# minfenli/refnerf-pl

Measured on AMD Instinct MI355X. Metric: ray-samples/s (4096 rays x 128 samples x 2 levels, Ref-NeRF Blender, eval forward), higher is better.
Workload: dtype f16x2; 1 GPU; blender_refnerf.gin, 4096 rays x 128 samples, 2-level, Model.__call__ eval forward with compute_extras + full ray_history; rays_per_gpu=4096, total_rays=4096, samples_per_level=128, parallelism=ray-tile dp1, n_ranks_seen=1, hip_graph_replay=False

## Files before the change

refnerf-pl_amd/csrc/refnerf_device_math.h:

```cpp
#pragma once
#include <hip/hip_runtime.h>

#include "refnerf_detmath.h"
#include "refnerf_layout.h"
#include "refnerf_ide_tables.h"

namespace rn {

constexpr float EPS32 = 1.1920928955078125e-07f;
constexpr float HALF_PI_F = 1.57079637050628662109375f;
constexpr float T100PI = 314.159271240234375f;
constexpr float LOG3_F = 1.09861228466033935546875f;
constexpr float LOG2E_F = 1.44269504088896341f;
constexpr float LN2_F = 0.69314718055994531f;
constexpr float INV_2PI_F = 0.15915494309189535f;


__device__ __forceinline__ float clip01(float x) { return fminf(fmaxf(x, 0.0f), 1.0f); }

__device__ __forceinline__ float s_to_t(float s, float nearv, float farv) {
  float a = s * farv;
  float b = (1.0f - s) * nearv;
  return a + b;
}
// ... 58 lines not shown

__device__ __forceinline__ void cast_sample(const float o[3], const float d[3], float radius, float t0,
                                            float t1, int ray_shape, float lmean[3], float lvar[3]) {
  float t_mean, t_var, r_var;
  frustum_moments(radius, t0, t1, ray_shape, t_mean, t_var, r_var);
  float dms = fmaxf(1e-10f, (d[0] * d[0] + d[1] * d[1]) + d[2] * d[2]);
  float mean[3], cd[3];
#pragma unroll
  for (int i = 0; i < 3; ++i) {
    mean[i] = d[i] * t_mean + o[i];
    float d_outer = d[i] * d[i];
    float null_outer = 1.0f - d[i] * (d[i] / dms);
    cd[i] = t_var * d_outer + r_var * null_outer;
  }
  lmean[0] = -mean[2]; lmean[1] = -mean[1]; lmean[2] = -mean[0];
  lvar[0] = cd[2]; lvar[1] = cd[1]; lvar[2] = cd[0];
}

__device__ __forceinline__ void cast_sample_full(const float o[3], const float d[3], float radius, float t0, float t1, int ray_shape,
                                                 float mean[3], float cov[9]) {
  float t_mean, t_var, r_var;
  frustum_moments(radius, t0, t1, ray_shape, t_mean, t_var, r_var);
  const float dms = fmaxf(1e-10f, (d[0] * d[0] + d[1] * d[1]) + d[2] * d[2]);
#pragma unroll
  for (int i = 0; i < 3; ++i) {
    mean[i] = d[i] * t_mean + o[i];
#pragma unroll
    for (int k = 0; k < 3; ++k) {
      const float d_outer = d[i] * d[k];
      const float null_outer = (i == k ? 1.0f : 0.0f) - d[i] * (d[k] / dms);
      cov[3 * i + k] = t_var * d_outer + r_var * null_outer;
    }
  }
}
__device__ __forceinline__ void lift_onto(const float mean[3], const float cov[9], const float b[3], float &lm, float &lv) {
  lm = fmaf(mean[2], b[2], fmaf(mean[1], b[1], mean[0] * b[0]));
  float acc = 0.0f;
#pragma unroll
  for (int i = 0; i < 3; ++i) {
    const float cb = fmaf(cov[3 * i + 2], b[2], fmaf(cov[3 * i + 1], b[1], cov[3 * i] * b[0]));
    acc = (i == 0) ? b[0] * cb : acc + b[i] * cb;
  }
  lv = acc;
}

__device__ __forceinline__ float safe_arg(float x) {
  if (fabsf(x) < T100PI) return x;
  float m = fmodf(x, T100PI);
  if (m != 0.0f && m < 0.0f) m += T100PI;
  return m;
}

__device__ __forceinline__ void quadrant_reduce(float a, float &r, int &q) {
  const float k = __builtin_rintf(a * 0.636619772367581343f);
  r = fmaf(-k, 7.54978995489188216e-8f, fmaf(-k, 4.837512969970703125e-4f, fmaf(-k, 1.5703125f, a)));
  q = (int)k;
}
__device__ __forceinline__ float sin_reduced(float a) {
  float r; int q;
  quadrant_reduce(a, r, q);
  const float r2 = r * r;
  const float s = fmaf(fmaf(fmaf(-1.9515295891e-4f, r2, 8.3321608736e-3f), r2, -1.6666654611e-1f) * r2, r, r);
  const float c = fmaf(fmaf(fmaf(2.443315711809948e-5f, r2, -1.388731625493765e-3f), r2, 4.166664568298827e-2f) * r2, r2, fmaf(-0.5f, r2, 1.0f));
  const float v = (q & 1) ? c : s;
  return (q & 2) ? -v : v;
}
__device__ __forceinline__ float cos_reduced(float a) {
  float r; int q;
  quadrant_reduce(a, r, q);
  const float r2 = r * r;
  const float s = fmaf(fmaf(fmaf(-1.9515295891e-4f, r2, 8.3321608736e-3f), r2, -1.6666654611e-1f) * r2, r, r);
  const float c = fmaf(fmaf(fmaf(2.443315711809948e-5f, r2, -1.388731625493765e-3f), r2, 4.166664568298827e-2f) * r2, r2, fmaf(-0.5f, r2, 1.0f));
  const float v = (q & 1) ? s : c;
  return ((q + 1) & 2) ? -v : v;
}
__device__ __forceinline__ float safe_arg_exact(float x) {
  const float q = __builtin_floorf(fmaf(x, 1.0f / T100PI, 3e-4f));
  float r = fmaf(-q, T100PI, x);
  r = (r < 0.0f) ? r + T100PI : r;
  return (fabsf(x) < T100PI) ? x : r;
}
__device__ __forceinline__ float ipe_feature_split(float lm, float lv, int j, int cos_block) {
  const float sc = __builtin_ldexpf(1.0f, j), sc2 = __builtin_ldexpf(1.0f, 2 * j);
  float x = lm * sc;
  if (cos_block) x = x + HALF_PI_F;
  const float e = __builtin_amdgcn_exp2f((-0.5f * LOG2E_F) * (lv * sc2));
  return e * sin_reduced(safe_arg_exact(x));
}

template <bool FAST = false>
__device__ __forceinline__ float ipe_feature(float lm, float lv, int j, int cos_block) {
  float sc = __builtin_ldexpf(1.0f, j), sc2 = __builtin_ldexpf(1.0f, 2 * j);
  if (FAST) {
    float r = (lm * sc) * INV_2PI_F;
    if (cos_block) r = r + 0.25f;
    r = __builtin_amdgcn_fractf(r);
    float e = __builtin_amdgcn_exp2f((-0.5f * LOG2E_F) * (lv * sc2));
    return e * __builtin_amdgcn_sinf(r);
  }
  float x = lm * sc;
  if (cos_block) x = x + HALF_PI_F;
  float e = expf(-0.5f * (lv * sc2));
  return e * sinf(safe_arg(x));
}

template <bool FAST> __device__ __forceinline__ float m_exp(float x) {
  if (FAST) return __builtin_amdgcn_exp2f(x * LOG2E_F);
  return expf(x);
}
template <bool FAST> __device__ __forceinline__ float m_log(float x) {
  if (FAST) return __builtin_amdgcn_logf(x) * LN2_F;
  return logf(x);
}
template <bool FAST> __device__ __forceinline__ float m_div(float a, float b) {
  if (FAST) return a * __builtin_amdgcn_rcpf(b);
  return a / b;
}
template <bool FAST> __device__ __forceinline__ float softplus_m(float x) {
  if (FAST) return x > 20.0f ? x : m_log<true>(1.0f + m_exp<true>(x));
  return x > 20.0f ? x : log1pf(expf(x));
}
template <bool FAST> __device__ __forceinline__ float sigmoid_m(float x) { return m_div<FAST>(1.0f, 1.0f + m_exp<FAST>(-x)); }
__device__ __forceinline__ float softplus_t(float x) { return softplus_m<false>(x); }
__device__ __forceinline__ float sigmoid_t(float x) { return sigmoid_m<false>(x); }

template <bool FAST = false>
__device__ __forceinline__ float linear_to_srgb(float x) {
  float srgb0 = (float)(323.0 / 25.0) * x;
  float pw = FAST ? __builtin_amdgcn_exp2f(__builtin_amdgcn_logf(fmaxf(EPS32, x)) * (float)(5.0 / 12.0))
                  : powf(fmaxf(EPS32, x), (float)(5.0 / 12.0));
  float srgb1 = FAST ? (211.0f * pw - 11.0f) * (1.0f / 200.0f) : (211.0f * pw - 11.0f) / 200.0f;
  return (x <= 0.0031308f) ? srgb0 : srgb1;
}

template <bool FAST = false, typename Emit>
__device__ __forceinline__ void ide_eval(float x, float y, float z, float kappa_inv, int part, Emit emit) {
  float att1 = m_exp<FAST>(-1.0f * kappa_inv), att2 = m_exp<FAST>(-3.0f * kappa_inv), att4 = m_exp<FAST>(-10.0f * kappa_inv);
  float att8 = m_exp<FAST>(-36.0f * kappa_inv), att16 = m_exp<FAST>(-136.0f * kappa_inv);
  float pr = 1.0f, pi = 0.0f;
#pragma unroll
  for (int m = 0; m <= 16; ++m) {
    if (m > 0) { float nr = pr * x - pi * y; float ni = pr * y + pi * x; pr = nr; pi = ni; }
    const float pw = part ? pi : pr;
    float tm2 = 0.0f, tm1 = IDE_C[m];
#pragma unroll
    for (int l = m; l <= 16; ++l) {
      float tl;
      if (l == m) tl = IDE_C[m];
      else { tl = IDE_A[m][l] * (z * tm1 - IDE_B[m][l] * tm2); tm2 = tm1; tm1 = tl; }
      if (l == 1) emit(0 + m, pw * (tl * att1));
      if (l == 2) emit(2 + m, pw * (tl * att2));
      if (l == 4) emit(5 + m, pw * (tl * att4));
      if (l == 8) emit(10 + m, pw * (tl * att8));
      if (l == 16) emit(19 + m, pw * (tl * att16));
    }
  }
}

template <bool FAST = false, bool REDUCED = false, typename Emit>
__device__ __forceinline__ void posenc_eval(float x, float y, float z, int part, Emit emit) {
  const float d[3] = {x, y, z};
  const float half_pi = (float)(0.5 * 3.14159265358979323846);
#pragma unroll
  for (int q = 0; q < IDE_TERMS; ++q) {
    float v = 0.0f;
    if (q < 3 && part == 0) v = d[q];
// ... 105 lines not shown
```

refnerf-pl_amd/csrc/refnerf_level_bf16.h:

```cpp
#pragma once
#include <type_traits>

#include "refnerf_level_common.h"

namespace rn {

typedef short v2s __attribute__((ext_vector_type(2)));

struct MmBf16 {
  typedef __bf16 t;
  typedef t v8 __attribute__((ext_vector_type(8)));
  typedef t v2 __attribute__((ext_vector_type(2)));
  static __device__ __forceinline__ v16f mfma(v8 a, v8 b, v16f c) { return __builtin_amdgcn_mfma_f32_32x32x16_bf16(a, b, c, 0, 0, 0); }
};
struct MmF16 {
  typedef _Float16 t;
  typedef t v8 __attribute__((ext_vector_type(8)));
  typedef t v2 __attribute__((ext_vector_type(2)));
  static __device__ __forceinline__ v16f mfma(v8 a, v8 b, v16f c) { return __builtin_amdgcn_mfma_f32_32x32x16_f16(a, b, c, 0, 0, 0); }
};
template <typename MM>
__device__ __forceinline__ unsigned cvt_pk_mm(float lo, float hi) {
  typename MM::v2 r = __builtin_convertvector((v2f){lo, hi}, typename MM::v2);
  return __builtin_bit_cast(unsigned, r);
// ... 338 lines not shown
      RN_STAMPW(A, 3 + phase * 8);

      if (phase == 0) bf_layer<MM, BF_LDS8, BF_IPE_REAL_KS>(p, ar, 0, R0, bn, R0);
      else bf_layer<MM, BF_BNLDS, BF_DIR_REAL_KS>(p, ar, 0, R0, bn, R0);
      RN_STAMPW(A, 4 + phase * 8);
#pragma unroll 1
      for (int it = 0; it < 4; ++it) {
        const int second = (it == 2) ? (phase ? 2 : 1) : 0;
        bf_layer<MM, BF_REG, 0>(p, ar, second, R0, bn, R1);
        if (it < 3) bf_layer<MM, BF_REG, 0>(p, ar, 0, R1, bn, R0);
      }
      RN_STAMPW(A, 5 + phase * 8);
      if (phase == 0) {
#pragma unroll
        for (int ob = 0; ob < 5; ++ob) {
          v16f acc;
          bf_slice<MM, BF_REG, 0>(p, ar, 0, R1, bn, acc);
          if (ob < 4) pack_acc<MM, false>(acc, bn[2 * ob], bn[2 * ob + 1]);
          else {
            int cb = col + 4 * h * BT;
            asm volatile("" : "+v"(cb));
#pragma unroll
            for (int rr = 0; rr < 8; ++rr) {
              int row = (rr & 3) + 8 * (rr >> 2) + 4 * h;
              if (row < HD_ROWS) HD[((rr & 3) + 8 * (rr >> 2)) * BT + cb] = acc[rr];
            }
          }
        }
        wave_sync();
        RN_STAMPW(A, 6);
      } else {
        v16f acc;
        bf_slice<MM, BF_REG, 0>(p, ar, 0, R1, bn, acc);
        float raw_rgb[3];
#pragma unroll
        for (int i = 0; i < 3; ++i) raw_rgb[i] = __shfl(acc[i], n, 64);
        int g_w, rl_w, si_w; bool valid;
        locate(g_w, rl_w, si_w, valid);
        int lane_w = lane, pass_w = pass0;
        asm volatile("" : "+v"(lane_w), "+s"(pass_w));
        if (valid && h == 0) {
          SampleHeads sh;
          load_heads(sh);
          colour_store<ENC_FAST, NPS_EVAL, PSM>(A, sh, raw_rgb, PS, PX, n_tot, g_w, col);
        }
        wave_sync();
        history_flush<NPS_EVAL, PSM>(A, PS, PX, n_tot, pass_w + wave * 32, wave * 32, (size_t)ray0 * N + pass_w + wave * 32, lane_w);
        RN_STAMPW(A, 14);
      }
    }
    __builtin_amdgcn_wave_barrier();
    pass_epilogue();
  }
  asm volatile("s_waitcnt vmcnt(0)" ::: "memory");
  __syncthreads();
  RN_STAMPW(A, 15);
#ifdef REFNERF_PROF_WAITS
  if (A.prof && blockIdx.x == 0 && lane == 0) { A.prof[wave * 32 + 20] = p.t_vm; A.prof[wave * 32 + 21] = p.t_bar; }
#endif

  if constexpr (!RINGPS) composite_phase<BF_NW, true, NPS_EVAL>(A, TD, XP, PS, n_tot, ray0, wave, lane, reinterpret_cast<float *>(WB), NRM);
  RN_STAMPW(A, 16);
}

#ifndef REFNERF_SECONDARY_TU
__global__ __launch_bounds__(BF_NTHREADS) void level_fwd_bf16(const LevelArgs A) { level_fwd_mm<MmBf16>(A); }
__global__ __launch_bounds__(BF_NTHREADS) void level_fwd_f16(const LevelArgs A) { level_fwd_mm<MmF16>(A); }
__global__ __launch_bounds__(BF_NTHREADS) void level_fwd_bf16_ring(const LevelArgs A) { level_fwd_mm<MmBf16, true>(A); }
__global__ __launch_bounds__(BF_NTHREADS) void level_fwd_f16_ring(const LevelArgs A) { level_fwd_mm<MmF16, true>(A); }
#endif

typedef unsigned v2uu __attribute__((ext_vector_type(2)));

__device__ __forceinline__ unsigned pk_f16(float lo, float hi) { return cvt_pk_mm<MmF16>(lo, hi); }
__device__ __forceinline__ void split_pair_f16(float x0, float x1, unsigned &hi, unsigned &lo) {
  hi = pk_f16(x0, x1);
  asm("" : "+v"(hi));
  const MmF16::v2 hv = __builtin_bit_cast(MmF16::v2, hi);
  const _Float16 h0 = hv[0], h1 = hv[1];
  lo = pk_f16(x0 - (float)h0, x1 - (float)h1);
}
typedef _Float16 sq_v8 __attribute__((ext_vector_type(8)));
constexpr int SQ_NF = 4;
struct SqAcc { v4f t0, t1; };
template <int KIND> constexpr int sq_nm() { return KIND == SQ_X ? 18 : (KIND == SQ_BN ? 32 : 24); }
template <int KIND> constexpr int sq_np() { return KIND == SQ_X ? 12 : 16; }
template <int KIND> constexpr int sq_step(int j) { return KIND == SQ_BN ? j / 4 : (KIND == SQ_SC ? j / 3 : j / 6); }
template <int KIND> constexpr int sq_piece(int j) {
  if (KIND == SQ_BN) return 2 * (j / 4) + (j & 1);
  if (KIND == SQ_SC) return 2 * (j / 3) + ((j % 3) == 1 ? 1 : 0);
  return 4 * (j / 6) + ((j % 6) < 4 ? (j % 6) : (j % 6) - 4);
}
template <int KIND> constexpr bool sq_lo(int j) { return KIND == SQ_BN ? (j & 3) >= 2 : (KIND == SQ_SC ? (j % 3) == 2 : (j % 6) >= 4); }
template <int KIND> constexpr int sq_tile(int j) { return KIND == SQ_SC ? 0 : (KIND == SQ_BN ? (j & 1) : ((j % 6) & 1)); }
template <int KIND> constexpr int sq_release(int j) {
  if (KIND == SQ_BN) return (j & 3) >= 2 ? 2 * (j / 4) + ((j & 3) - 2) : -1;
  if (KIND == SQ_SC) return (j % 3) == 1 ? 2 * (j / 3) + 1 : ((j % 3) == 2 ? 2 * (j / 3) : -1);
  const int jj = j % 6, sl = j / 6;
  return jj == 2 ? 4 * sl + 2 : (jj == 3 ? 4 * sl + 3 : (jj == 4 ? 4 * sl : (jj == 5 ? 4 * sl + 1 : -1)));
}
template <int KIND, bool PRE, typename Hook = NoHook>
__device__ __forceinline__ void sq_chunk(Pipe &p, sq_v8 (&fr)[SQ_NF], const v4uu (&in)[16], SqAcc &acc, SqAcc &nacc, Hook &&hook = Hook(), int adv = BF_CHUNK_BYTES) {
  constexpr int NM = sq_nm<KIND>(), NP = sq_np<KIND>();
  constexpr int RDV = NM / 2 - 1;
  const char *w = p.wbuf + p.cur_off;
  const char *cur = w + 1024 + p.lane * 16;
  const char *nxt = p.wbuf + p.nxt_off + 1024 + p.lane * 16;
  sq_v8 xb[2];
  if (KIND == SQ_X) { xb[0] = lds_frag<MmF16>(p.xps); xb[1] = lds_frag<MmF16>(p.xps + (BT / 2) * 16); }
  __builtin_amdgcn_sched_barrier(0);
#pragma unroll
  for (int j = 0; j < NM; ++j) {
    const int sl = sq_step<KIND>(j);
    sq_v8 b;
    if (KIND == SQ_X) b = xb[sq_lo<KIND>(j) ? 1 : 0];
    else b = __builtin_bit_cast(sq_v8, in[2 * ((KIND == SQ_B ? 4 : 0) + sl) + (sq_lo<KIND>(j) ? 1 : 0)]);
    if (sq_tile<KIND>(j)) acc.t1 = __builtin_amdgcn_mfma_f32_16x16x32_f16(fr[sq_piece<KIND>(j) % SQ_NF], b, acc.t1, 0, 0, 0);
    else acc.t0 = __builtin_amdgcn_mfma_f32_16x16x32_f16(fr[sq_piece<KIND>(j) % SQ_NF], b, acc.t0, 0, 0, 0);
    const int rel = sq_release<KIND>(j);
    if (rel >= 0) {
      const int q = rel + SQ_NF;
      fr[rel % SQ_NF] = (q < NP) ? lds_frag<MmF16>(cur + q * 1024) : lds_frag<MmF16>(nxt + (q - NP) * 1024);
    }
    hook(j);
    if (KIND == SQ_X) {
      if ((j % 6) == 3 && sl + 1 < 3) xb[0] = lds_frag<MmF16>(p.xps + (sl + 1) * (4 * BT * 16));
      if ((j % 6) == 5 && sl + 1 < 3) xb[1] = lds_frag<MmF16>(p.xps + (sl + 1) * (4 * BT * 16) + (BT / 2) * 16);
    }
    if (j == RDV) {
      RN_RENDEZVOUS(p);
      issue_chunk<true>(p, p.fil_off, 0);
      if (PRE) {
        const v4f *bp = reinterpret_cast<const v4f *>(p.wbuf + p.nxt_off + (p.lane >> 4) * 16);
        nacc.t0 = bp[0];
        nacc.t1 = bp[4];
      }
    }
    if (j == RDV + 4) issue_chunk<true>(p, p.fil_off, 1);
    if (j == RDV + 8) issue_chunk<true>(p, p.fil_off, 2, adv);
    __builtin_amdgcn_sched_barrier(0);
  }
  ring_rotate(p);
}
__device__ __forceinline__ void sq_epi_piece(const SqAcc &a, int q, v4uu &oh, v4uu &ol) {
  const float y0 = q == 0 ? a.t0[0] : (q == 1 ? a.t0[2] : (q == 2 ? a.t1[0] : a.t1[2]));
  const float y1 = q == 0 ? a.t0[1] : (q == 1 ? a.t0[3] : (q == 2 ? a.t1[1] : a.t1[3]));
  const float x0 = (y0 < 0.0f) ? 0.0f : y0, x1 = (y1 < 0.0f) ? 0.0f : y1;
  unsigned hi, lo;
  split_pair_f16(x0, x1, hi, lo);
  oh[q] = hi;
  ol[q] = lo;
}
template <bool LAYER0>
__device__ __forceinline__ void sq_layer(Pipe &p, sq_v8 (&fr)[SQ_NF], SqAcc (&accs)[2], bool skip, const v4uu (&in)[16], v4uu (&out)[16]) {
#pragma unroll
  for (int ob = 0; ob < 8; ++ob) {
    SqAcc &acc = accs[(ob + 1) & 1];
    SqAcc &prev = accs[ob & 1];
    auto hook = [&](int j) {
      if (ob == 0 || j >= 8 || (j & 1)) return;
      sq_epi_piece(prev, j >> 1, out[2 * ob - 2], out[2 * ob - 1]);
    };
    if constexpr (LAYER0) sq_chunk<SQ_X, true>(p, fr, in, acc, prev, hook);
    else {
      sq_chunk<SQ_A, false>(p, fr, in, acc, prev, hook);
      sq_chunk<SQ_B, true>(p, fr, in, acc, prev);
      if (skip) sq_chunk<SQ_X, true>(p, fr, in, acc, prev);
    }
  }
#pragma unroll
  for (int q = 0; q < 4; ++q) sq_epi_piece(accs[0], q, out[14], out[15]);
  __builtin_amdgcn_sched_barrier(0);
}
__device__ __forceinline__ void sq_bias_now(const Pipe &p, SqAcc &acc) {
  const v4f *bp = reinterpret_cast<const v4f *>(p.wbuf + p.cur_off + (p.lane >> 4) * 16);
  acc.t0 = bp[0];
  acc.t1 = bp[4];
}

template <typename MM, int KIND0, int REAL0>
__device__ __forceinline__ void dir_layer(Pipe &p, typename MM::v8 (&a)[AF], int second, const v4uu (&in)[16], const v4uu (&bn)[8], v4uu (&out)[16], int adv6 = BF_CHUNK_BYTES) {
#pragma unroll
  for (int ob = 0; ob < 8; ++ob) {
    v16f acc;
    bf_chunk<MM, KIND0, REAL0, true, true>(p, a, in, bn, acc, NoHook(), ob == 6 ? adv6 : BF_CHUNK_BYTES);
    if constexpr (KIND0 == BF_REG) {
      if (second == 2) bf_chunk<MM, BF_BNLDS, BF_DIR_REAL_KS, false, true>(p, a, in, bn, acc);
    }
    pack_acc<MM, true>(acc, out[2 * ob], out[2 * ob + 1]);
    __builtin_amdgcn_sched_barrier(0);
  }
}

template <bool RINGPS = false>
__device__ __forceinline__ void level_fwd_split(const LevelArgs &A) {
  typedef MmF16 MM;
  constexpr int PSM = RINGPS ? BF_PS_RING - 1 : 0;
  typedef typename MM::v8 v8mm;
  typedef typename MM::t mm_t;
  extern __shared__ __attribute__((aligned(16))) float smem[];
  const refnerf_level_cfg &cfg = A.cfg;
  const int N = cfg.n_samples;
  const int tid = threadIdx.x, lane = tid & 63;
  const int wave = __builtin_amdgcn_readfirstlane(tid >> 6);
  const int rpw = A.rpw;
  const int ray0 = blockIdx.x * rpw;
  const int n_tot = rpw * N;
  const int n_pass = (n_tot + BT - 1) / BT;

  char *WB = reinterpret_cast<char *>(smem);
  char *Xb = WB + BF_RING_BYTES;
  float *HD = reinterpret_cast<float *>(Xb + BF_X_BYTES);
  float *TD = HD + HD_ROWS * BT;
  float *XP = TD + rpw * (N + 1);
  float *PS = XP + rpw * (N + 1);
  float *PX = PS + (RINGPS ? BF_PS_RING : n_tot) * NPS_EVAL;
  float *NRM = PX + 3 * BT;
  const float *RY = NRM + 8;

  const int h = lane >> 5, n = lane & 31;
  const int col = wave * 32 + n;

  Pipe p;
  pipe_stream_init(p, A.packed, n_pass * SPPACKED.chunks_per_pass, wave, lane);
  p.wbuf = WB;
  p.xp = Xb + (h * BT + col) * 16;
  p.xps = Xb + ((lane >> 4) * BT + wave * 16 + (lane & 15)) * 16;
  p.cur_off = 0; p.nxt_off = BF_CHUNK_BYTES; p.fil_off = 2 * BF_CHUNK_BYTES;
  p.lane = lane; p.wave = wave; p.h = h;
  p.t_vm = 0; p.t_bar = 0;
  RN_STAMPW(A, 0);
#ifdef REFNERF_PROF_WAITS
  if (A.prof && blockIdx.x == (gridDim.x >> 1) && lane == 0) A.prof[wave * 32 + 22] = (long long)__builtin_amdgcn_s_memrealtime();
#endif
  issue_chunk<true>(p, p.cur_off);
  issue_chunk<true>(p, p.nxt_off);

  resample_phase<BF_NW, true>(A, reinterpret_cast<float *>(Xb), TD, NRM, ray0, wave, lane);
#pragma clang loop unroll(disable)
  for (int rl = wave; rl < rpw; rl += BF_NW) {
    const int ray = ray0 + rl;
    if (ray >= A.R) break;
    float *RYw = NRM + 8 + rl * 12;
    if (lane < 10) {
      const float val = lane < 3 ? A.rays.d_origins[(size_t)ray * 3 + lane]
                      : lane < 6 ? A.rays.d_directions[(size_t)ray * 3 + lane - 3]
                      : lane < 9 ? A.rays.d_viewdirs[(size_t)ray * 3 + lane - 6] : A.rays.d_radii[ray];
      RYw[lane] = val;
      const float dx = __shfl(val, 3, 64), dy = __shfl(val, 4, 64), dz = __shfl(val, 5, 64);
      if (lane == 0) NRM[rl] = sqrtf((dx * dx + dy * dy) + dz * dz);
    }
  }
  RN_STAMPW(A, 1);
  asm volatile("s_waitcnt vmcnt(0)" ::: "memory");
  __syncthreads();
  RN_STAMPW(A, 2);

  if (wave >= BF_NW / 2) __builtin_amdgcn_s_setprio(1);
  v4uu R0[16], R1[16];
  sq_v8 ar[SQ_NF];
#pragma unroll
  for (int d = 0; d < SQ_NF; ++d) ar[d] = lds_frag<MM>(WB + 1024 + lane * 16 + d * 1024);

  for (int pass0 = 0; pass0 < n_tot; pass0 += BT) {
    int lane_v = lane;
    asm volatile("" : "+v"(lane_v));
    p.lane_off = (unsigned)(wave * 3072 + lane_v * 16);
    auto locate = [&](int &g, int &rl, bool &valid) {
      int col_l = col, pass_l = pass0;
      asm volatile("" : "+v"(col_l), "+s"(pass_l));
      g = pass_l + col_l;
      rl = g / N;
      valid = (g < n_tot) && (ray0 + rl < A.R);
    };
    auto pass_epilogue = [&]() {
      if constexpr (RINGPS) {
        __syncthreads();
        const int end = (pass0 + BT < n_tot) ? pass0 + BT : n_tot;
        int td_o = (int)(TD - smem), xp_o = (int)(XP - smem), ps_o = (int)(PS - smem), nrm_o = (int)(NRM - smem), lane_e = lane, pass_e = pass0;
        int ntot_e = n_tot, ray0_e = ray0, wave_e = wave;
        asm volatile("" : "+s"(td_o), "+s"(xp_o), "+s"(ps_o), "+s"(nrm_o), "+v"(lane_e), "+s"(pass_e), "+s"(ntot_e), "+s"(ray0_e), "+s"(wave_e));
        composite_phase<BF_NW, false, NPS_EVAL, PSM>(A, smem + td_o, smem + xp_o, smem + ps_o, ntot_e, ray0_e, wave_e, lane_e, nullptr, smem + nrm_o,
                                                     pass_e / N, end / N);
      }
    };
    {
      const int g0 = pass0 + wave * 32;
      if (g0 >= n_tot || ray0 + g0 / N >= A.R) { idle_pass<true>(p); pass_epilogue(); continue; }
    }
    auto load_heads = [&](SampleHeads &sh) {
      int g, rl; bool valid;
      locate(g, rl, valid);
      int ci = col, ro = (valid ? rl : 0) * 12;
      asm volatile("" : "+v"(ci), "+v"(ro));
      float v[3], gp[3], raw_dif[3], raw_tint[3];
#pragma unroll
      for (int i = 0; i < 3; ++i) {
        v[i] = RY[ro + 6 + i];
        gp[i] = HD[(1 + i) * BT + ci];
        raw_dif[i] = HD[(5 + i) * BT + ci];
        raw_tint[i] = HD[(8 + i) * BT + ci];
      }
      sample_heads<false>(cfg, HD[0 * BT + ci], gp, HD[4 * BT + ci], raw_dif, raw_tint, v, sh);
    };

    v4uu bn0[4];
    auto heads = [&](auto RUN, v4uu (&bn)[8]) {
      constexpr int run = decltype(RUN)::value;
      SqAcc ha[2];
      sq_bias_now(p, ha[1]);
#pragma unroll
      for (int ob = 0; ob < 5; ++ob) {
        SqAcc &acc = ha[(ob + 1) & 1];
        if (ob < 4) {
          sq_chunk<SQ_BN, true>(p, ar, R1, acc, ha[ob & 1], NoHook(), (run == 0 && ob == 2) ? SP_ADV_REWIND : BF_CHUNK_BYTES);
#pragma unroll
          for (int e = 0; e < 4; ++e) {
            const unsigned pk = e == 0 ? pk_f16(acc.t0[0], acc.t0[1]) : (e == 1 ? pk_f16(acc.t0[2], acc.t0[3])
                              : (e == 2 ? pk_f16(acc.t1[0], acc.t1[1]) : pk_f16(acc.t1[2], acc.t1[3])));
            if (run == 0) bn0[ob][e] = pk;
            else {
              const v2uu r = __builtin_amdgcn_permlane16_swap(bn0[ob][e], pk, false, false);
              bn[2 * ob][e] = r[0];
              bn[2 * ob + 1][e] = r[1];
            }
          }
        } else {
          sq_chunk<SQ_SC, false>(p, ar, R1, acc, ha[ob & 1]);
          const int bq = lane_v >> 4;
          int csl = wave * 32 + 16 * run + (lane_v & 15) + 4 * bq * BT;
          asm volatile("" : "+v"(csl));
#pragma unroll
          for (int i = 0; i < 4; ++i)
            if (4 * bq + i < HD_ROWS) HD[i * BT + csl] = acc.t0[i];
        }
      }
      wave_sync();
    };
    typedef std::integral_constant<int, 0> Run0;
    typedef std::integral_constant<int, 1> Run1;

#pragma unroll 1
    for (int phase = 0; phase < 2; ++phase) {
#pragma unroll
      for (int e = 0; e < 16; ++e) { R0[e] = (v4uu){0, 0, 0, 0}; R1[e] = (v4uu){0, 0, 0, 0}; }
      {
      const int i16 = lane_v & 15, part = lane_v >> 4;
      const int hb = part >> 1, qq = part & 1;
      const int cs = wave * 32 + 16 * phase + i16;
      const int gs = pass0 + cs;
      const int rls = gs / N, sis = gs - rls * N;
      const bool vs = (gs < n_tot) && (ray0 + rls < A.R);
      float o[3], d[3];
      const float *ry = RY + (vs ? rls : 0) * 12;
#pragma unroll
      for (int i = 0; i < 3; ++i) { o[i] = ry[i]; d[i] = ry[3 + i]; }
      const float radius = ry[9];
      const float *td = TD + (vs ? rls : 0) * (N + 1);
      const float t0 = td[vs ? sis : 0], t1 = td[vs ? sis + 1 : 1];
      float lm[3], lv[3];
      cast_sample(o, d, radius, t0, t1, cfg.ray_shape, lm, lv);
      if (cfg.disable_integration) { lv[0] = 0.0f; lv[1] = 0.0f; lv[2] = 0.0f; }
      char *xw = Xb + (wave * 16 + i16) * 16;
      RN_STAMPW(A, 17);
#pragma clang loop unroll(disable)
      for (int t = 0; t < 12; ++t) {
        unsigned whi, wlo;
        {
          float f[2];
#pragma unroll
          for (int u = 0; u < 2; ++u) {
            const int kk = 2 * t + u;
            const int jj = kk / 3, b3 = kk - 3 * jj;
            const float m = b3 == 0 ? lm[0] : (b3 == 1 ? lm[1] : lm[2]);
            const float v = b3 == 0 ? lv[0] : (b3 == 1 ? lv[1] : lv[2]);
            f[u] = ipe_feature_split(m, v, 8 * qq + jj, hb);
          }
          split_pair_f16(f[0], f[1], whi, wlo);
        }
        char *dst = xw + (6 * hb + 3 * qq + (t >> 2)) * BT * 16 + (t & 3) * 4;
        *reinterpret_cast<unsigned *>(dst) = whi;
        *reinterpret_cast<unsigned *>(dst + (BT / 2) * 16) = wlo;
      }
      }
      RN_STAMPW(A, 18);
      wave_sync();
      RN_STAMPW(A, 3 + phase * 4);
      if (phase == 0) {
#pragma unroll
        for (int d = AF; d < SQ_NF; ++d) ar[d] = lds_frag<MM>(p.wbuf + p.cur_off + 1024 + lane_v * 16 + d * 1024);
      }
      SqAcc accs[2];
      sq_bias_now(p, accs[1]);
      sq_layer<true>(p, ar, accs, false, R0, R0);
      RN_STAMPW(A, 4 + phase * 4);
#pragma unroll 1
      for (int it = 0; it < 4; ++it) {
        sq_layer<false>(p, ar, accs, it == 2, R0, R1);
        if (it < 3) sq_layer<false>(p, ar, accs, false, R1, R0);
      }
      RN_STAMPW(A, 5 + phase * 4);
      if (phase == 0) {
        v4uu none[8];
        heads(Run0(), none);
        RN_STAMPW(A, 6);
      }
    }
    v4uu bn[8];
    heads(Run1(), bn);
    RN_STAMPW(A, 10);
#pragma unroll
    for (int e = 0; e < 16; ++e) { R0[e] = (v4uu){0, 0, 0, 0}; R1[e] = (v4uu){0, 0, 0, 0}; }
    {
    const int h4 = RINGPS ? (fresh_lane() >> 5) : h;
    char *xs = Xb + col * 16;
    {
      SampleHeads sh;
      load_heads(sh);
      float ide[40];
#pragma unroll
      for (int q = 36; q < 40; ++q) ide[q] = 0.0f;
      if (cfg.dir_enc == REFNERF_DIRENC_POSENC) posenc_eval<false, true>(sh.refd[0], sh.refd[1], sh.refd[2], h4, [&](int q, float val) { ide[q] = val; });
      else ide_eval<false>(sh.refd[0], sh.refd[1], sh.refd[2], sh.rough, h4, [&](int q, float val) { ide[q] = val; });
      if (h4 == 0) ide[36] = sh.dot;
#pragma unroll
      for (int q = 0; q < 5; ++q) {
        v8mm pk;
#pragma unroll
        for (int e = 0; e < 8; ++e) pk[e] = (mm_t)ide[q * 8 + e];
        *reinterpret_cast<v8mm *>(xs + (5 * h4 + q) * BT * 16) = pk;
      }
    }
    wave_sync();
    RN_STAMPW(A, 11);
    v8mm (&ad)[AF] = reinterpret_cast<v8mm (&)[AF]>(ar);
    dir_layer<MM, BF_BNLDS, BF_DIR_REAL_KS>(p, ad, 0, R0, bn, R0);
    RN_STAMPW(A, 12);
#pragma unroll 1
    for (int it = 0; it < 4; ++it) {
      dir_layer<MM, BF_REG, 0>(p, ad, (it == 2) ? 2 : 0, R0, bn, R1, it == 3 ? SP_ADV_WRAP : BF_CHUNK_BYTES);
      if (it < 3) dir_layer<MM, BF_REG, 0>(p, ad, 0, R1, bn, R0);
    }
    RN_STAMPW(A, 13);
    v16f acc;
    bf_chunk<MM, BF_REG, 0, true, true>(p, ad, R1, bn, acc);
    float raw_rgb[3];
    const int lane6 = RINGPS ? fresh_lane() : lane;
    const int n6 = RINGPS ? (lane6 & 31) : n, h6 = RINGPS ? (lane6 >> 5) : h;
#pragma unroll
    for (int i = 0; i < 3; ++i) raw_rgb[i] = __shfl(acc[i], n6, 64);
    int g_w, rl_w; bool valid;
    locate(g_w, rl_w, valid);
    int lane_w = lane6, pass_w = pass0;
    asm volatile("" : "+v"(lane_w), "+s"(pass_w));
    if (valid && h6 == 0) {
      SampleHeads sh;
      load_heads(sh);
      colour_store<false, NPS_EVAL, PSM, true, RINGPS>(A, sh, raw_rgb, PS, PX, n_tot, g_w, RINGPS ? wave * 32 + n6 : col);
    }
    wave_sync();
    history_flush<NPS_EVAL, PSM>(A, PS, PX, n_tot, pass_w + wave * 32, wave * 32, (size_t)ray0 * N + pass_w + wave * 32, lane_w);
    RN_STAMPW(A, 14);
    }
    __builtin_amdgcn_wave_barrier();
    pass_epilogue();
  }
  asm volatile("s_waitcnt vmcnt(0)" ::: "memory");
  __syncthreads();
  RN_STAMPW(A, 15);
#ifdef REFNERF_PROF_WAITS
  if (A.prof && blockIdx.x == (gridDim.x >> 1) && lane == 0) {
    A.prof[wave * 32 + 20] = p.t_vm; A.prof[wave * 32 + 21] = p.t_bar;
    A.prof[wave * 32 + 23] = (long long)__builtin_amdgcn_s_memrealtime();
  }
#endif
  if constexpr (!RINGPS) composite_phase<BF_NW, false, NPS_EVAL>(A, TD, XP, PS, n_tot, ray0, wave, lane, reinterpret_cast<float *>(WB), NRM);
  RN_STAMPW(A, 16);
}

#ifndef REFNERF_SECONDARY_TU
__global__ __launch_bounds__(BF_NTHREADS) void level_fwd_f16x2(const LevelArgs A) { level_fwd_split<false>(A); }
__global__ __launch_bounds__(BF_NTHREADS) void level_fwd_f16x2_ring(const LevelArgs A) { level_fwd_split<true>(A); }
#endif

__device__ __forceinline__ int ipe_col_of_kprime(int kp) { return kp; }

}
```

refnerf-pl_amd/csrc/refnerf_level_common.h:

```cpp
#pragma once
#include <hip/hip_runtime.h>

#include "refnerf_hip.h"
#include "refnerf_device_math.h"
#include "refnerf_layout.h"

namespace rn {

typedef float v16f __attribute__((ext_vector_type(16)));
typedef float v4f __attribute__((ext_vector_type(4)));
typedef unsigned int v4u __attribute__((ext_vector_type(4)));

constexpr int NTHREADS = 256;

typedef __bf16 v8bf __attribute__((ext_vector_type(8)));
typedef unsigned v4uu __attribute__((ext_vector_type(4)));
typedef __bf16 v2bf __attribute__((ext_vector_type(2)));
typedef float v2f __attribute__((ext_vector_type(2)));
__device__ __forceinline__ unsigned cvt_pk_bf16(float lo, float hi) {
  v2bf r = __builtin_convertvector((v2f){lo, hi}, v2bf);
  return __builtin_bit_cast(unsigned, r);
}

constexpr int HD_ROWS = 12;
// ... 208 lines not shown
    for (int k = lane; k <= N; k += 64) {
      float s = sd[k];
      if (A.out.d_sdist) A.out.d_sdist[(size_t)ray * (N + 1) + k] = s;
      sd[k] = s_to_t(s, nearv, farv, A.cfg.raydist);
    }
  }
}

struct SampleHeads {
  float density, rough, dot;
  float tint[3], raw_dif[3], npred[3], gp[3], refd[3];
  float normals[3] = {0.0f, 0.0f, 0.0f};
};
template <bool FAST = false>
__device__ __forceinline__ void sample_heads(const refnerf_level_cfg &cfg, float raw_density, const float gp[3],
                                             float raw_rough, const float raw_dif[3], const float raw_tint[3],
                                             const float v[3], SampleHeads &s) {
#pragma unroll
  for (int i = 0; i < 3; ++i) { s.gp[i] = gp[i]; s.raw_dif[i] = raw_dif[i]; s.tint[i] = sigmoid_m<FAST>(raw_tint[i]); }
  float n2 = fmaxf((gp[0] * gp[0] + gp[1] * gp[1]) + gp[2] * gp[2], EPS32);
  float nrm = sqrtf(n2);
#pragma unroll
  for (int i = 0; i < 3; ++i) s.npred[i] = -m_div<FAST>(gp[i], nrm);
  s.density = softplus_m<FAST>(raw_density + cfg.density_bias);
  s.rough = softplus_m<FAST>(raw_rough + cfg.roughness_bias);
  float w3[3] = {-v[0], -v[1], -v[2]};
  float dot = (s.npred[0] * w3[0] + s.npred[1] * w3[1]) + s.npred[2] * w3[2];
#pragma unroll
  for (int i = 0; i < 3; ++i) s.refd[i] = (2.0f * dot) * s.npred[i] - w3[i];
  s.dot = (s.npred[0] * v[0] + s.npred[1] * v[1]) + s.npred[2] * v[2];
}

template <int PSM>
__device__ __forceinline__ int ps_row(int g) { return PSM ? (g & PSM) : g; }

template <bool FAST = false, int NP = NPS_TRAIN, int PSM = 0, bool FAST_SRGB = FAST, bool PAD_HERE = false>
__device__ __forceinline__ void colour_store(const LevelArgs &A, const SampleHeads &s, const float raw_rgb[3],
                                             float *PS, float *PX, int n_tot, int g_sample, int gcol) {
  const int g = ps_row<PSM>(g_sample);
  const refnerf_level_cfg &cfg = A.cfg;
  float spec_lin[3], dif_lin[3], rgb[3], dif[3], spc[3];
#pragma unroll
  for (int i = 0; i < 3; ++i) {
    float sg = sigmoid_m<FAST>(cfg.rgb_premultiplier * raw_rgb[i] + cfg.rgb_bias);
    dif_lin[i] = sigmoid_m<FAST>(s.raw_dif[i] - LOG3_F);
    spec_lin[i] = s.tint[i] * sg;
    rgb[i] = spec_lin[i] + dif_lin[i];
  }
  if (cfg.srgb_mapping) {
    if (cfg.srgb_mapping_normalization) {
      float norm = fmaxf(fmaxf(fmaxf(rgb[0], rgb[1]), rgb[2]), 1.0f);
#pragma unroll
      for (int i = 0; i < 3; ++i) rgb[i] = m_div<FAST>(rgb[i], norm);
    }
#pragma unroll
    for (int i = 0; i < 3; ++i) {
      rgb[i] = clip01(linear_to_srgb<FAST_SRGB>(rgb[i]));
      dif[i] = clip01(linear_to_srgb<FAST_SRGB>(dif_lin[i]));
      spc[i] = clip01(linear_to_srgb<FAST_SRGB>(spec_lin[i]));
    }
  } else {
#pragma unroll
    for (int i = 0; i < 3; ++i) { dif[i] = dif_lin[i]; spc[i] = spec_lin[i]; }
  }
  float pad = cfg.rgb_padding;
  if (PAD_HERE) asm volatile("" : "+s"(pad));
  const float pad_scale = (float)(1.0 + 2.0 * (double)pad);
#pragma unroll
  for (int i = 0; i < 3; ++i) rgb[i] = rgb[i] * pad_scale - pad;
  PS[g * NP + PS_DENSITY] = s.density;
  PS[g * NP + PS_ROUGH] = s.rough;
#pragma unroll
  for (int i = 0; i < 3; ++i) {
    PS[g * NP + PS_RGB + i] = rgb[i];
    PS[g * NP + PS_DIF + i] = dif[i];
    PS[g * NP + PS_SPC + i] = spc[i];
    PS[g * NP + PS_NPRED + i] = s.npred[i];
    PS[g * NP + PS_TINT + i] = s.tint[i];
    if (NP > PS_NORMALS) PS[g * NP + PS_NORMALS + i] = s.normals[i];
    PX[gcol * 3 + i] = s.gp[i];
  }
}

__device__ __forceinline__ void hist_store(float *p, float v) { __builtin_nontemporal_store(v, p); }
constexpr int AUX_NT = 2;

template <int NP = NPS_TRAIN, int PSM = 0>
__device__ __forceinline__ void history_flush(const LevelArgs &A, const float *PS, const float *PX, int n_tot, int gw0, int gcol0,
                                              size_t gs0, int lane) {
  const size_t total = (size_t)A.R * A.cfg.n_samples;
  auto vec3 = [&](float *dst, int slot) {
    if (!dst) return;
#pragma unroll
    for (int it = 0; it < 2; ++it) {
      const int f = lane + 64 * it;
      const int smp = f / 3, c = f - 3 * smp;
      if (f < 96 && gw0 + smp < n_tot && gs0 + smp < total) hist_store(dst + gs0 * 3 + f, PS[ps_row<PSM>(gw0 + smp) * NP + slot + c]);
    }
  };
  auto scal = [&](float *dst, int slot) {
    if (dst && lane < 32 && gw0 + lane < n_tot && gs0 + lane < total) hist_store(dst + gs0 + lane, PS[ps_row<PSM>(gw0 + lane) * NP + slot]);
  };
  scal(A.out.d_density, PS_DENSITY);
  scal(A.out.d_roughness, PS_ROUGH);
  vec3(A.out.d_rgb, PS_RGB);
  vec3(A.out.d_diffuse, PS_DIF);
  vec3(A.out.d_specular, PS_SPC);
  vec3(A.out.d_normals_pred, PS_NPRED);
  if (A.out.d_grad_pred) {
#pragma unroll
    for (int it = 0; it < 2; ++it) {
      const int f = lane + 64 * it;
      const int smp = f / 3;
      if (f < 96 && gw0 + smp < n_tot && gs0 + smp < total) hist_store(A.out.d_grad_pred + gs0 * 3 + f, PX[gcol0 * 3 + f]);
    }
  }
  vec3(A.out.d_tint, PS_TINT);
  if (NP > PS_NORMALS && A.cfg.training) vec3(A.out.d_normals, PS_NORMALS);
}

template <int NW = 4, bool FAST = false, int NP = NPS_TRAIN, int PSM = 0>
__device__ __forceinline__ void composite_phase(const LevelArgs &A, const float *TD, float *XP, float *PS, int n_tot,
                                                int ray0, int wave, int lane, float *wscr, const float *NRM,
                                                int rl_begin = 0, int rl_end = -1) {
  const refnerf_level_cfg &cfg = A.cfg;
  const int N = cfg.n_samples, rpw = A.rpw;
  if (rl_end < 0) rl_end = rpw;
  #pragma clang loop unroll(disable)
  for (int rl = rl_begin + wave; rl < rl_end; rl += NW) {
    const int ray = ray0 + rl;
    if (ray >= A.R) break;
    const float *td = TD + rl * (N + 1);
    const int base = rl * N;
    const int C = (N + 63) / 64;
    const int i0 = lane * C;
    float norm;
    if (FAST) norm = NRM[rl];
    else {
      float dx = A.rays.d_directions[(size_t)ray * 3], dy = A.rays.d_directions[(size_t)ray * 3 + 1], dz = A.rays.d_directions[(size_t)ray * 3 + 2];
      norm = sqrtf((dx * dx + dy * dy) + dz * dz);
    }
    auto wref = [&](int i) -> float & { return PS[ps_row<PSM>(base + i) * NP + PS_DENSITY]; };
    auto rec = [&](int i, int slot) { return PS[ps_row<PSM>(base + i) * NP + slot]; };
    double local = 0.0;
    #pragma clang loop unroll(disable)
    for (int q = 0; q < C; ++q) {
      int i = i0 + q;
      if (i < N) {
        float dd = wref(i) * ((td[i + 1] - td[i]) * norm);
        if (!(cfg.opaque_background && i == N - 1)) local += (double)dd;
      }
    }
    double incl = wave_scan_incl(local, lane);
    double cum = incl - local;
    float acc = 0, s_rgb[3] = {0, 0, 0}, s_dif[3] = {0, 0, 0}, s_spc[3] = {0, 0, 0}, s_np[3] = {0, 0, 0}, s_tn[3] = {0, 0, 0};
    float s_nm[3] = {0, 0, 0};
    float s_dist = 0, s_rgh = 0, s_logd = 0;
    double wlocal = 0.0;
    #pragma clang loop unroll(disable)
    for (int q = 0; q < C; ++q) {
      int i = i0 + q;
      if (i < N) {
        float dd = wref(i) * ((td[i + 1] - td[i]) * norm);
        if (cfg.opaque_background && i == N - 1) dd = INFINITY;
        float alpha = 1.0f - m_exp<FAST>(-dd);
        float trans = m_exp<FAST>(-(float)cum);
// ... 150 lines not shown
```

Baseline: 270.2 million ray-samples/s.

## Split colour epilogue across wave halves and streamline IPE feature generation

IPE feature generation now carries the frequency scales incrementally instead of recomputing the power-of-two scale and selecting components per term. The layer-0 input fragments are preloaded from LDS into a separate register array using a new SQ_XR chunk kind, and that array is cleared afterwards. Head values are stored to PS earlier, where they are already loaded. The final colour store is split so both wave halves each compute one sigmoid branch and combine them through a cross-half shuffle, instead of one half reloading heads and doing all the work. The aim is to cut redundant ALU and load work and idle lanes in the epilogue, at the cost of extra register pressure and LDS reads of tint.

```diff
diff --git a/refnerf-pl_amd/csrc/refnerf_device_math.h b/refnerf-pl_amd/csrc/refnerf_device_math.h
--- a/refnerf-pl_amd/csrc/refnerf_device_math.h
+++ b/refnerf-pl_amd/csrc/refnerf_device_math.h
@@ -164,6 +164,12 @@
 }
 __device__ __forceinline__ float ipe_feature_split(float lm, float lv, int j, int cos_block) {
   const float sc = __builtin_ldexpf(1.0f, j), sc2 = __builtin_ldexpf(1.0f, 2 * j);
+  float x = lm * sc;
+  if (cos_block) x = x + HALF_PI_F;
+  const float e = __builtin_amdgcn_exp2f((-0.5f * LOG2E_F) * (lv * sc2));
+  return e * sin_reduced(safe_arg_exact(x));
+}
+__device__ __forceinline__ float ipe_feature_split_sc(float lm, float lv, float sc, float sc2, int cos_block) {
   float x = lm * sc;
   if (cos_block) x = x + HALF_PI_F;
   const float e = __builtin_amdgcn_exp2f((-0.5f * LOG2E_F) * (lv * sc2));
diff --git a/refnerf-pl_amd/csrc/refnerf_level_bf16.h b/refnerf-pl_amd/csrc/refnerf_level_bf16.h
--- a/refnerf-pl_amd/csrc/refnerf_level_bf16.h
+++ b/refnerf-pl_amd/csrc/refnerf_level_bf16.h
@@ -444,9 +444,11 @@
 }
 typedef _Float16 sq_v8 __attribute__((ext_vector_type(8)));
 constexpr int SQ_NF = 4;
+constexpr int SQ_XR = 11;
+static_assert(SQ_XR != SQ_A && SQ_XR != SQ_B && SQ_XR != SQ_X && SQ_XR != SQ_BN && SQ_XR != SQ_SC, "a kind of its own");
 struct SqAcc { v4f t0, t1; };
-template <int KIND> constexpr int sq_nm() { return KIND == SQ_X ? 18 : (KIND == SQ_BN ? 32 : 24); }
-template <int KIND> constexpr int sq_np() { return KIND == SQ_X ? 12 : 16; }
+template <int KIND> constexpr int sq_nm() { return (KIND == SQ_X || KIND == SQ_XR) ? 18 : (KIND == SQ_BN ? 32 : 24); }
+template <int KIND> constexpr int sq_np() { return (KIND == SQ_X || KIND == SQ_XR) ? 12 : 16; }
 template <int KIND> constexpr int sq_step(int j) { return KIND == SQ_BN ? j / 4 : (KIND == SQ_SC ? j / 3 : j / 6); }
 template <int KIND> constexpr int sq_piece(int j) {
   if (KIND == SQ_BN) return 2 * (j / 4) + (j & 1);
@@ -523,7 +525,7 @@
       if (ob == 0 || j >= 8 || (j & 1)) return;
       sq_epi_piece(prev, j >> 1, out[2 * ob - 2], out[2 * ob - 1]);
     };
-    if constexpr (LAYER0) sq_chunk<SQ_X, true>(p, fr, in, acc, prev, hook);
+    if constexpr (LAYER0) sq_chunk<SQ_XR, true>(p, fr, in, acc, prev, hook);
     else {
       sq_chunk<SQ_A, false>(p, fr, in, acc, prev, hook);
       sq_chunk<SQ_B, true>(p, fr, in, acc, prev);
@@ -533,6 +535,13 @@
 #pragma unroll
   for (int q = 0; q < 4; ++q) sq_epi_piece(accs[0], q, out[14], out[15]);
   __builtin_amdgcn_sched_barrier(0);
+}
+__device__ __forceinline__ void sq_load_ipe_frags(const Pipe &p, v4uu (&in)[16]) {
+#pragma unroll
+  for (int s = 0; s < 3; ++s) {
+    in[2 * s] = __builtin_bit_cast(v4uu, lds_frag<MmF16>(p.xps + s * (4 * BT * 16)));
+    in[2 * s + 1] = __builtin_bit_cast(v4uu, lds_frag<MmF16>(p.xps + s * (4 * BT * 16) + (BT / 2) * 16));
+  }
 }
 __device__ __forceinline__ void sq_bias_now(const Pipe &p, SqAcc &acc) {
   const v4f *bp = reinterpret_cast<const v4f *>(p.wbuf + p.cur_off + (p.lane >> 4) * 16);
@@ -650,8 +659,8 @@
       const int g0 = pass0 + wave * 32;
       if (g0 >= n_tot || ray0 + g0 / N >= A.R) { idle_pass<true>(p); pass_epilogue(); continue; }
     }
-    auto load_heads = [&](SampleHeads &sh) {
-      int g, rl; bool valid;
+    auto load_heads = [&](SampleHeads &sh, int &g, bool &valid) {
+      int rl;
       locate(g, rl, valid);
       int ci = col, ro = (valid ? rl : 0) * 12;
       asm volatile("" : "+v"(ci), "+v"(ro));
@@ -725,24 +734,28 @@
       if (cfg.disable_integration) { lv[0] = 0.0f; lv[1] = 0.0f; lv[2] = 0.0f; }
       char *xw = Xb + (wave * 16 + i16) * 16;
       RN_STAMPW(A, 17);
+      float sc = qq ? 256.0f : 1.0f, sc2 = qq ? 65536.0f : 1.0f;
+      char *xq = xw + (6 * hb + 3 * qq) * BT * 16;
 #pragma clang loop unroll(disable)
-      for (int t = 0; t < 12; ++t) {
-        unsigned whi, wlo;
-        {
+      for (int dp = 0; dp < 4; ++dp) {
+        const float sc_odd = sc * 2.0f, sc2_odd = sc2 * 4.0f;
+#pragma unroll
+        for (int a = 0; a < 3; ++a) {
           float f[2];
 #pragma unroll
           for (int u = 0; u < 2; ++u) {
-            const int kk = 2 * t + u;
-            const int jj = kk / 3, b3 = kk - 3 * jj;
-            const float m = b3 == 0 ? lm[0] : (b3 == 1 ? lm[1] : lm[2]);
-            const float v = b3 == 0 ? lv[0] : (b3 == 1 ? lv[1] : lv[2]);
-            f[u] = ipe_feature_split(m, v, 8 * qq + jj, hb);
+            const int k6 = 2 * a + u, odd = k6 / 3, b3 = k6 - 3 * odd;
+            f[u] = ipe_feature_split_sc(lm[b3], lv[b3], odd ? sc_odd : sc, odd ? sc2_odd : sc2, hb);
           }
+          unsigned whi, wlo;
           split_pair_f16(f[0], f[1], whi, wlo);
+          const int t = 3 * dp + a;
+          char *dst = xq + (t >> 2) * BT * 16 + (t & 3) * 4;
+          *reinterpret_cast<unsigned *>(dst) = whi;
+          *reinterpret_cast<unsigned *>(dst + (BT / 2) * 16) = wlo;
         }
-        char *dst = xw + (6 * hb + 3 * qq + (t >> 2)) * BT * 16 + (t & 3) * 4;
-        *reinterpret_cast<unsigned *>(dst) = whi;
-        *reinterpret_cast<unsigned *>(dst + (BT / 2) * 16) = wlo;
+        sc *= 4.0f;
+        sc2 *= 16.0f;
       }
       }
       RN_STAMPW(A, 18);
@@ -754,7 +767,10 @@
       }
       SqAcc accs[2];
       sq_bias_now(p, accs[1]);
-      sq_layer<true>(p, ar, accs, false, R0, R0);
+      sq_load_ipe_frags(p, R1);
+      sq_layer<true>(p, ar, accs, false, R1, R0);
+#pragma unroll
+      for (int e = 0; e < 6; ++e) R1[e] = (v4uu){0, 0, 0, 0};
       RN_STAMPW(A, 4 + phase * 4);
 #pragma unroll 1
       for (int it = 0; it < 4; ++it) {
@@ -778,7 +794,9 @@
     char *xs = Xb + col * 16;
     {
       SampleHeads sh;
-      load_heads(sh);
+      int g4; bool valid4;
+      load_heads(sh, g4, valid4);
+      if (valid4 && h4 == 0) heads_store<NPS_EVAL, PSM>(sh, PS, PX, g4, RINGPS ? wave * 32 + (fresh_lane() & 31) : col);
       float ide[40];
 #pragma unroll
       for (int q = 36; q < 40; ++q) ide[q] = 0.0f;
@@ -815,10 +833,15 @@
     locate(g_w, rl_w, valid);
     int lane_w = lane6, pass_w = pass0;
     asm volatile("" : "+v"(lane_w), "+s"(pass_w));
-    if (valid && h6 == 0) {
-      SampleHeads sh;
-      load_heads(sh);
-      colour_store<false, NPS_EVAL, PSM, true, RINGPS>(A, sh, raw_rgb, PS, PX, n_tot, g_w, RINGPS ? wave * 32 + n6 : col);
+    if (valid) {
+      int ci = RINGPS ? wave * 32 + n6 : col, pr = ps_row<PSM>(g_w) * NPS_EVAL;
+      asm volatile("" : "+v"(ci), "+v"(pr));
+      float tint[3], raw_dif[3];
+#pragma unroll
+      for (int i = 0; i < 3; ++i) { tint[i] = PS[pr + PS_TINT + i]; raw_dif[i] = HD[(5 + i) * BT + ci]; }
+      int half = h6;
+      asm volatile("" : "+v"(half));
+      colour_store_halves<NPS_EVAL, PSM, true>(A, half, tint, raw_dif, raw_rgb, PS, g_w);
     }
     wave_sync();
     history_flush<NPS_EVAL, PSM>(A, PS, PX, n_tot, pass_w + wave * 32, wave * 32, (size_t)ray0 * N + pass_w + wave * 32, lane_w);
diff --git a/refnerf-pl_amd/csrc/refnerf_level_common.h b/refnerf-pl_amd/csrc/refnerf_level_common.h
--- a/refnerf-pl_amd/csrc/refnerf_level_common.h
+++ b/refnerf-pl_amd/csrc/refnerf_level_common.h
@@ -314,6 +314,54 @@
   }
 }
 
+template <int NP, int PSM>
+__device__ __forceinline__ void heads_store(const SampleHeads &s, float *PS, float *PX, int g_sample, int gcol) {
+  const int g = ps_row<PSM>(g_sample);
+  PS[g * NP + PS_DENSITY] = s.density;
+  PS[g * NP + PS_ROUGH] = s.rough;
+#pragma unroll
+  for (int i = 0; i < 3; ++i) {
+    PS[g * NP + PS_NPRED + i] = s.npred[i];
+    PS[g * NP + PS_TINT + i] = s.tint[i];
+    PX[gcol * 3 + i] = s.gp[i];
+  }
+}
+template <int NP, int PSM, bool PAD_HERE>
+__device__ __forceinline__ void colour_store_halves(const LevelArgs &A, int half, const float tint[3], const float raw_dif[3],
+                                                    const float raw_rgb[3], float *PS, int g_sample) {
+  const int g = ps_row<PSM>(g_sample);
+  const refnerf_level_cfg &cfg = A.cfg;
+  float own[3], rgb[3];
+#pragma unroll
+  for (int i = 0; i < 3; ++i) {
+    const float sg = sigmoid_m<false>(half ? raw_dif[i] - LOG3_F : cfg.rgb_premultiplier * raw_rgb[i] + cfg.rgb_bias);
+    own[i] = half ? sg : tint[i] * sg;
+  }
+#pragma unroll
+  for (int i = 0; i < 3; ++i) rgb[i] = own[i] + __shfl_xor(own[i], 32, 64);
+  if (cfg.srgb_mapping) {
+    if (cfg.srgb_mapping_normalization) {
+      float norm = fmaxf(fmaxf(fmaxf(rgb[0], rgb[1]), rgb[2]), 1.0f);
+#pragma unroll
+      for (int i = 0; i < 3; ++i) rgb[i] = m_div<false>(rgb[i], norm);
+    }
+#pragma unroll
+    for (int i = 0; i < 3; ++i) {
+      rgb[i] = clip01(linear_to_srgb<true>(rgb[i]));
+      own[i] = clip01(linear_to_srgb<true>(own[i]));
+    }
+  }
+  float pad = cfg.rgb_padding;
+  if (PAD_HERE) asm volatile("" : "+s"(pad));
+  const float pad_scale = (float)(1.0 + 2.0 * (double)pad);
+  const int own_slot = half ? PS_DIF : PS_SPC;
+#pragma unroll
+  for (int i = 0; i < 3; ++i) {
+    PS[g * NP + own_slot + i] = own[i];
+    if (!half) PS[g * NP + PS_RGB + i] = rgb[i] * pad_scale - pad;
+  }
+}
+
 __device__ __forceinline__ void hist_store(float *p, float v) { __builtin_nontemporal_store(v, p); }
 constexpr int AUX_NT = 2;
 
```

Result: faster. 273.1 million ray-samples/s, median of 6 (+1.1%).
